# impICNF/ContinuousNF.jl

Measured on AMD Instinct MI355X. Metric: ODE RHS-evals/sec (nvars=32, batch=8192, Tsit5), higher is better.
Workload: dtype f32 (products as six bf16 MFMA terms of exactly split operands, fp32 accumulate); 1 GPU; BASELINE configs[2]: RNODE nvars=32 naugs=0, MLP 32-128-128-32 tanh, batch 8192 per GPU, TrainMode Hutchinson VJP, Tsit5 tspan (0,1), adaptive reltol=sqrt(eps32) abstol=eps32; global_batch=8192, parallelism=columns sharded x1, kernel=mfma

## Files before the change

### continuousnf.jl_amd/csrc/cnf_step3.hip

```cpp
#include "cnf_step3_dev.h"
#include <mutex>

namespace s3 {
constexpr int NB = 32, P0 = 32, PH = 128;
constexpr int SX0 = 40, SXH = 136, SKZ = 264, SW2 = 132;
constexpr int W1T = 0;
constexpr int W3R = W1T + P0 * SXH;
constexpr int X0 = W3R + P0 * SXH;
constexpr int H1 = X0 + NB * SX0;
constexpr int H2 = H1 + NB * SXH;
constexpr int G1 = H2 + NB * SXH;
constexpr int G3 = G1 + NB * SXH;
constexpr int KZ = G3 + NB * SX0;
constexpr int RED = KZ + NB * SKZ;
constexpr int SC = RED + 3 * NB * 8;
constexpr int EPS = SC + NB * 24;
constexpr int BIAS = EPS + NB * SX0;
constexpr int MISC = BIAS + 2 * PH + P0;
constexpr int TOTAL = MISC + 64;
constexpr int STG = X0;
static_assert(STG + PH * SW2 <= RED, "the W2 staging image must not reach the scratch that the prologue uses");
constexpr int IMG_W2 = 0;
constexpr int IMG_W1T = IMG_W2 + PH * SW2;
constexpr int IMG_W3R = IMG_W1T + P0 * SXH;
// ... 1098 lines not shown
            }
            if (live && sown) {
                const f32x4 f1 = read_scalars();
                out[n_in] = f1.x; out[n_in + 1] = f1.y; out[n_in + 2] = f1.z;
                if (a.init_phase >= 0) norms(sc_get(0), sc_get(1), f1, 3);
            }
        }
        if (!single && live && zown) {
            const f32x4 ez = TS_BT1 * kz[0] + TS_BT2 * kz[1] + TS_BT3 * kz[2] + TS_BT4 * kz[3] + TS_BT5 * kz[4] +
                             TS_BT6 * kz[5] + TS_BT7 * kz[6];
#pragma unroll
            for (int c = 0; c < 4; ++c) {
                const float scl = fmaf(fmaxf(fabsf(uz[c]), fabsf(un[c])), reltol, abstol);
                const float x = c < nv ? hstep * ez[c] / scl : 0.f;
                errsum = fmaf(x, x, errsum);
                badcnt += (c < nv && !(fabsf(un[c]) <= 3.0e38f)) ? 1.f : 0.f;
            }
            const size_t gc = (size_t)(tile * 32 + 16 * hf + s) * D;
            if (nv >= 4) { st4_wide(Uout + gc + r0, un); st4_wide(K1out + gc + r0, kz[6]); }
            else { st4(Uout + gc + r0, un, nv); st4(K1out + gc + r0, kz[6], nv); }
        }
        if (!single && live && sown) {
            f32x4 ks[7];
#pragma unroll
            for (int j = 0; j < 6; ++j) ks[j] = sc_get(1 + j);
            const f32x4 us = sc_get(0);
            ks[6] = read_scalars();
            const f32x4 uns = us + hstep * stage_acc4<6>(ks);
            err_acc(errsum, badcnt, ks, us, uns, hstep, abstol, reltol, 3);
            const size_t gc = (size_t)(tile * 32 + 16 * hf + s) * D;
            float* Un = Uout + gc + n_in;
            float* K7 = K1out + gc + n_in;
            Un[0] = uns.x; Un[1] = uns.y; Un[2] = uns.z;
            K7[0] = ks[6].x; K7[1] = ks[6].y; K7[2] = ks[6].z;
        }
        s3_bar();
    }
    errsum = s3_wave_sum(errsum);
    badcnt = s3_wave_sum(badcnt);
    if (lane == 0) { msc[wave] = errsum; msc[16 + wave] = badcnt; }
    s3_bar();
    if (tid == 0) {
        float e = 0.f, b = 0.f;
        for (int w = 0; w < 8; ++w) { e += msc[w]; b += msc[16 + w]; }
        if (!single) {
            a.partials[2 * blockIdx.x] = e;
            a.partials[2 * blockIdx.x + 1] = b;
        } else if (a.init_phase >= 0) {
            __hip_atomic_store(a.partials + 2 * blockIdx.x, e, __ATOMIC_RELAXED, __HIP_MEMORY_SCOPE_AGENT);
            __hip_atomic_store(a.partials + 2 * blockIdx.x + 1, b, __ATOMIC_RELAXED, __HIP_MEMORY_SCOPE_AGENT);
            asm volatile("s_waitcnt vmcnt(0)" ::: "memory");
            const unsigned tk = __hip_atomic_fetch_add(a.ticket, 1u, __ATOMIC_RELAXED, __HIP_MEMORY_SCOPE_AGENT);
            msc[40] = (tk == gridDim.x - 1) ? 1.f : 0.f;
            if (tk == gridDim.x - 1) __hip_atomic_store(a.ticket, 0u, __ATOMIC_RELAXED, __HIP_MEMORY_SCOPE_AGENT);
        }
    }
    if (single && a.init_phase >= 0) {
        s3_bar();
        if (msc[40] != 0.f) {
            float q0 = 0.f, q1 = 0.f;
            for (int i = tid; i < (int)gridDim.x; i += 512) {
                q0 += __hip_atomic_load(a.partials + 2 * i, __ATOMIC_RELAXED, __HIP_MEMORY_SCOPE_AGENT);
                q1 += __hip_atomic_load(a.partials + 2 * i + 1, __ATOMIC_RELAXED, __HIP_MEMORY_SCOPE_AGENT);
            }
            q0 = s3_wave_sum(q0); q1 = s3_wave_sum(q1);
            if (lane == 0) { msc[wave] = q0; msc[16 + wave] = q1; }
            s3_bar();
            if (tid == 0) {
                float p0 = 0.f, p1 = 0.f;
                for (int w = 0; w < 8; ++w) { p0 += msc[w]; p1 += msc[16 + w]; }
                ctrl_phase(a.st_out, single - 1, p0, p1, a.n_total);
            }
        }
    }
}

namespace s3v {
constexpr int SKZ = 264;
constexpr int KZ = 0, RED = KZ + 32 * SKZ, SC = RED + 3 * 32 * 8, BIAS = SC + 32 * 24;
constexpr int MISC = BIAS + 2 * 128 + 32, FP_END = MISC + 64;
constexpr int WS = 256, WP = 32 * WS, WI = 3 * WP;
constexpr int NS = 64, NP = 32 * NS, NI = 3 * NP;
constexpr int H1G = FP_END * 4, H2G = H1G + WI, W3I = H2G + WI, W1TI = W3I + WI, X0S = W1TI + WI, G3S = X0S + NI;
constexpr int TOTAL_BYTES = G3S + NI;
static_assert(H1G % 16 == 0 && TOTAL_BYTES <= 160 * 1024, "LDS plan");
static_assert(WI == s3g::WI, "global image");
}

__global__ void __launch_bounds__(512, 2) k_step3b(MfmaArgs a, const char* __restrict__ imgb, int n_in, int norm_z,
                                                   int norm_j, const S3Tab tab, int single) {
    extern __shared__ __attribute__((aligned(16))) float lds[];
    char* ldsb = reinterpret_cast<char*>(lds);
    const float* img3 = reinterpret_cast<const float*>(imgb);
    S3_ARGS_UP_FRONT(a, imgb);
    const StepState* st = a.st;
    const int tid = threadIdx.x, lane = tid & 63, wave = __builtin_amdgcn_readfirstlane(tid >> 6);
    const int D = n_in + 3;
    const int s = lane & 15, q = lane >> 4;
    const int t = wave & 1, hf = (wave >> 1) & 1;
    const bool zown = wave < 4;
    const bool sown = !zown && t == 0 && q == 0;
    const int smp = 16 * hf + s;
    const int r0 = 16 * t + 4 * q;
    const int nv = n_in - r0;
#ifdef S3_STAMPS
    unsigned long long s3acc[36] = {0};
    unsigned long long s3last = __builtin_amdgcn_s_memtime();
    const unsigned long long s3start = s3last;
#endif
    const StepState* stw = s3_state_words(st);
    const int v_done = stw->done, v_cur = stw->cur;
    const float v_h = stw->h, v_abstol = stw->abstol, v_reltol = stw->reltol;
    const float* ppin = a.apply_ctrl ? a.partials_in : img3;
    const float2 pp = *reinterpret_cast<const float2*>(ppin + 2 * min(tid, (int)gridDim.x - 1));
    const int ntile = (a.B + 32 - 1) / 32;
    const bool wide = (n_in & 3) == 0;
    f32x4 ru[2], rk[2], re, rs[2][2];
    int ce = 0, cu = 0, cs = 0;
    {
        const int b0 = blockIdx.x * 32 + 16 * hf;
        const bool live = s < max(0, min(16, a.B - b0));
        const size_t gcol = (size_t)(b0 + s) * D;
        ce = live ? nv : 0; cu = (zown && live) ? nv : 0; cs = (sown && live) ? 3 : 0;
        re = ld4_issue_w(a.eps + (size_t)(b0 + s) * n_in + r0, ce, img3, wide);
#pragma unroll
        for (int c = 0; c < 2; ++c) {
            ru[c] = ld4_issue_w(a.U[c] + gcol + r0, cu, img3, wide);
            rk[c] = ld4_issue_w(a.K1[c] + gcol + r0, cu, img3, wide);
            rs[c][0] = ld3_issue(a.U[c] + gcol + n_in, cs, img3);
            rs[c][1] = ld3_issue(a.K1[c] + gcol + n_in, cs, img3);
        }
    }
    constexpr int NCI = 2 * s3v::WI / 16, NCB = (2 * 128 + 32) / 4;
    static_assert(NCI % 64 == 0, "whole wave instructions");
    typedef __attribute__((address_space(3))) char* lds_c;
    typedef const __attribute__((address_space(1))) char* glb_c;
    const f32x4 sgb = reinterpret_cast<const f32x4*>(imgb + s3g::BIASB)[min(tid, NCB - 1)];
    S3bOp wF1, wF2[4], wB3, wB2[4];
    {
        const char* fw = imgb + s3g::F32 + (size_t)wave * 10 * 2048 + 16 * lane;
        constexpr int AH = 5;
        f32x4 raw[10][2];
#pragma unroll
        for (int f = 0; f < AH; ++f) { raw[f][0] = *(const f32x4*)(fw + f * 2048); raw[f][1] = *(const f32x4*)(fw + f * 2048 + 1024); }
        __builtin_amdgcn_sched_barrier(0);
#pragma unroll
        for (int f = 0; f < 10; ++f) {
            if (f + AH < 10) {
                raw[f + AH][0] = *(const f32x4*)(fw + (f + AH) * 2048);
                raw[f + AH][1] = *(const f32x4*)(fw + (f + AH) * 2048 + 1024);
            }
            S3bOp o = s3b_split8(raw[f][0], raw[f][1]);
            s3b_pin(o);
            if (f == 0) wF1 = o; else if (f < 5) wF2[f - 1] = o; else if (f == 5) wB3 = o; else wB2[f - 6] = o;
            __builtin_amdgcn_sched_barrier(0);
        }
    }
#pragma unroll
    for (int i = 0; i < (NCI + 511) / 512; ++i) {
        const int c = 512 * i + 64 * wave;
        if (c < NCI)
            __builtin_amdgcn_global_load_lds((glb_c)(imgb + s3g::W3I + 16 * (c + lane)), (lds_c)(ldsb + s3v::W3I + 16 * c), 16, 0, 0);
    }
    float* sc = lds + s3v::SC + smp * 24;
    auto sc_get = [&](int j) { return f32x4{sc[3 * j], sc[3 * j + 1], sc[3 * j + 2], 0.f}; };
    auto sc_set = [&](int j, const f32x4& v) { sc[3 * j] = v.x; sc[3 * j + 1] = v.y; sc[3 * j + 2] = v.z; };
    __builtin_amdgcn_sched_barrier(0);
    S3T(23);
    __builtin_amdgcn_s_waitcnt(0x0F70);
    __builtin_amdgcn_sched_barrier(0);
    S3T(24);
    const int st_done = __builtin_amdgcn_readfirstlane(v_done), st_cur = __builtin_amdgcn_readfirstlane(v_cur);
    const float st_h = __int_as_float(__builtin_amdgcn_readfirstlane(__float_as_int(v_h)));
    const float st_abstol = __int_as_float(__builtin_amdgcn_readfirstlane(__float_as_int(v_abstol)));
    const float st_reltol = __int_as_float(__builtin_amdgcn_readfirstlane(__float_as_int(v_reltol)));
    if (st_done) {
        asm volatile("s_waitcnt vmcnt(0)" ::: "memory");
        if (a.apply_ctrl && blockIdx.x == 0 && tid == 0) { *a.st_out = *st; publish_mirror(a, *st); }
        return;
    }
    if (sown) {
        sc_set(2, ld4_mask(rs[0][0], cs)); sc_set(3, ld4_mask(rs[0][1], cs));
        sc_set(4, ld4_mask(rs[1][0], cs)); sc_set(5, ld4_mask(rs[1][1], cs));
    }
    f32x4 epsr = ld4_mask(re, ce);
    float* msc = lds + s3v::MISC;
    if (a.apply_ctrl) {
        float cp0 = tid < (int)gridDim.x ? pp.x : 0.f, cp1 = tid < (int)gridDim.x ? pp.y : 0.f;
        for (int i = tid + 512; i < (int)gridDim.x; i += 512) { cp0 += a.partials_in[2 * i]; cp1 += a.partials_in[2 * i + 1]; }
        cp0 = s3_wave_sum(cp0); cp1 = s3_wave_sum(cp1);
        if (lane == 0) { msc[wave] = cp0; msc[16 + wave] = cp1; }
    }
    if (tid < NCB) reinterpret_cast<f32x4*>(lds + s3v::BIAS)[tid] = sgb;
    s3_bar();
    S3T(25);
    int cur = st_cur;
    float hstep = st_h, abstol = st_abstol, reltol = st_reltol;
    if (a.apply_ctrl && tid == 0) {
        float p0 = 0.f, p1 = 0.f;
        for (int w = 0; w < 8; ++w) { p0 += msc[w]; p1 += msc[16 + w]; }
        StepState ns = *st;
        ctrl_after_step(&ns, p0, p1, a.n_total);
        if (blockIdx.x == 0) { *a.st_out = ns; publish_mirror(a, ns); }
        msc[32] = __int_as_float(ns.cur); msc[33] = ns.h; msc[34] = ns.abstol; msc[35] = ns.reltol;
        msc[36] = __int_as_float(ns.done);
    }
    S3T(26);
    s3_bar();
    S3T(27);
    if (a.apply_ctrl) {
        cur = __builtin_amdgcn_readfirstlane(__float_as_int(msc[32]));
        hstep = __int_as_float(__builtin_amdgcn_readfirstlane(__float_as_int(msc[33])));
        abstol = __int_as_float(__builtin_amdgcn_readfirstlane(__float_as_int(msc[34])));
        reltol = __int_as_float(__builtin_amdgcn_readfirstlane(__float_as_int(msc[35])));
        if (__float_as_int(msc[36])) return;
    }
    const int nstg = single ? 1 : 6;
    const float c21 = single == 1 ? 0.f : (single == 2 ? 1.f : TS_A21);
    const float* Uin = cur ? a.U[1] : a.U[0];
    const float* K1in = cur ? a.K1[1] : a.K1[0];
    float* Uout = cur ? a.U[0] : a.U[1];
    float* K1out = cur ? a.K1[0] : a.K1[1];

    float errsum = 0.f, badcnt = 0.f;
    auto red8 = [&](int kind) {
        const float* r = lds + s3v::RED + (kind * 32 + smp) * 8;
        const f32x4 a_ = *(const f32x4*)r, b_ = *(const f32x4*)(r + 4);
        return ((a_.x + a_.y) + (a_.z + a_.w)) + ((b_.x + b_.y) + (b_.z + b_.w));
    };
    auto read_scalars = [&]() {
        const float e2 = red8(0), ld = red8(1), n2 = red8(2);
        return f32x4{ld, norm_z ? __builtin_sqrtf(e2) : 0.f, norm_j ? __builtin_sqrtf(n2) : 0.f, 0.f};
    };
    float* redw = lds + s3v::RED + smp * 8 + 4 * t + q;
    const int wb_rd = s * s3v::WS + 16 * (q ^ s);
    const int wb_wr = s * s3v::WS + 16 * ((2 * wave + (q >> 1)) ^ s) + 8 * (q & 1);
    constexpr int HBW = 16 * s3v::WS;
    const char* nrA = ldsb + (zown ? s3v::W3I : s3v::W1TI) + 16 * t * s3v::WS;
    const char* nrB = ldsb + (zown ? s3v::H2G : s3v::H1G) + 16 * hf * s3v::WS;
    const int nsw = (-(s >> 2)) & 3;
    const int nw = smp * s3v::NS + 16 * ((2 * t + (q >> 1)) ^ nsw) + 8 * (q & 1);
    char* x0w = ldsb + s3v::X0S + nw;
    char* g3w = ldsb + s3v::G3S + nw;
    const int nb_rd = s * s3v::NS + 16 * (q ^ nsw);
    constexpr int HBN = 16 * s3v::NS;
    float* rkw = lds + s3v::KZ + smp * s3v::SKZ + r0;
    float* kzw = rkw + 64;
    const float* bias = lds + s3v::BIAS;
    const f32x4 zero4 = {0.f, 0.f, 0.f, 0.f};

    S3T(20);
    auto tile_in = [&](const f32x4& uz, f32x4 k1z) {
        if (single == 1) { k1z = zero4; if (sown) sc_set(1, k1z); }
        if (zown) {
            s3b_store4(x0w, s3v::NP, uz + (hstep * c21) * k1z);
            *(f32x4*)rkw = uz;
            *(f32x4*)(rkw + 32) = k1z;
#pragma unroll
            for (int j = 0; j < 6; ++j) *(f32x4*)(kzw + 32 * j) = zero4;
        }
    };
    if (sown) { sc_set(0, sc_get(cur ? 4 : 2)); sc_set(1, sc_get(cur ? 5 : 3)); }
    tile_in(ld4_mask(cur ? ru[1] : ru[0], cu), ld4_mask(cur ? rk[1] : rk[0], cu));
    for (int tile = blockIdx.x; tile < ntile; tile += gridDim.x) {
        const int b0 = tile * 32 + 16 * hf;
        const bool live = s < max(0, min(16, a.B - b0));
        const size_t gcol = (size_t)(b0 + s) * D;
        if (tile != (int)blockIdx.x) {
            ce = live ? nv : 0; cu = (zown && live) ? nv : 0; cs = (sown && live) ? 3 : 0;
            const f32x4 e_ = ld4_issue_w(a.eps + (size_t)(b0 + s) * n_in + r0, ce, img3, wide);
            const f32x4 u_ = ld4_issue_w(Uin + gcol + r0, cu, img3, wide), k_ = ld4_issue_w(K1in + gcol + r0, cu, img3, wide);
            const f32x4 s0 = ld3_issue(Uin + gcol + n_in, cs, img3), s1 = ld3_issue(K1in + gcol + n_in, cs, img3);
            epsr = ld4_mask(e_, ce);
            if (sown) { sc_set(0, ld4_mask(s0, cs)); sc_set(1, ld4_mask(s1, cs)); }
            tile_in(ld4_mask(u_, cu), ld4_mask(k_, cu));
        }
        s3_bar();
        S3T(21);

        constexpr bool S3B_RECORDS = false;
        constexpr bool S3B_COND = false;
        float* const dmpw = nullptr; const size_t dmp_stride = 0;
        (void)dmpw; (void)dmp_stride;
#include "cnf_step3b_eval.inc"
        if (single) {
            float* out = (single == 1 ? a.du : a.Ks0) + (size_t)(tile * 32 + 16 * hf + s) * D;
            auto norms = [&](const f32x4& u4, const f32x4& f0, const f32x4& f1, int nvalid) {
#pragma unroll
                for (int c = 0; c < 4; ++c) {
                    if (c < nvalid) {
                        const float sk = fmaf(fabsf(u4[c]), reltol, abstol);
                        if (single == 1) {
                            const float x = u4[c] / sk, y = f1[c] / sk;
                            errsum = fmaf(x, x, errsum); badcnt = fmaf(y, y, badcnt);
                        } else {
                            const float x = (f1[c] - f0[c]) / sk;
                            errsum = fmaf(x, x, errsum);
                        }
                    }
                }
            };
            if (live && zown) {
                const f32x4 f1 = *(const f32x4*)kzw;
                st4(out + r0, f1, nv);
                if (a.init_phase >= 0) norms(*(const f32x4*)rkw, *(const f32x4*)(rkw + 32), f1, nv);
            }
            if (live && sown) {
                const f32x4 f1 = read_scalars();
                out[n_in] = f1.x; out[n_in + 1] = f1.y; out[n_in + 2] = f1.z;
                if (a.init_phase >= 0) norms(sc_get(0), sc_get(1), f1, 3);
            }
        }
        if (!single && live && zown) {
            const f32x4 k7z = *(const f32x4*)(kzw + 32 * 5), uz_ = *(const f32x4*)rkw;
            const f32x4 un = s3b_load4(x0w, s3v::NP);
            f32x4 ez = TS_BT1 * *(const f32x4*)(rkw + 32) + TS_BT7 * k7z;
            ez += TS_BT2 * *(const f32x4*)(kzw) + TS_BT3 * *(const f32x4*)(kzw + 32) + TS_BT4 * *(const f32x4*)(kzw + 64) +
                  TS_BT5 * *(const f32x4*)(kzw + 96) + TS_BT6 * *(const f32x4*)(kzw + 128);
#pragma unroll
            for (int c = 0; c < 4; ++c) {
                const float scl = fmaf(fmaxf(fabsf(uz_[c]), fabsf(un[c])), reltol, abstol);
                const float x = c < nv ? hstep * ez[c] / scl : 0.f;
                errsum = fmaf(x, x, errsum);
                badcnt += (c < nv && !(fabsf(un[c]) <= 3.0e38f)) ? 1.f : 0.f;
            }
            const size_t gc = (size_t)(tile * 32 + 16 * hf + s) * D;
            float* Un = Uout + gc + r0;
            float* K7 = K1out + gc + r0;
            if (nv >= 4) { st4_wide(Un, un); st4_wide(K7, k7z); }
            else { st4(Un, un, nv); st4(K7, k7z, nv); }
        }
        if (!single && live && sown) {
            f32x4 ks[7];
#pragma unroll
            for (int j = 0; j < 6; ++j) ks[j] = sc_get(1 + j);
            const f32x4 us = sc_get(0);
            ks[6] = read_scalars();
            const f32x4 uns = us + hstep * stage_acc4<6>(ks);
            err_acc(errsum, badcnt, ks, us, uns, hstep, abstol, reltol, 3);
            const size_t gc = (size_t)(tile * 32 + 16 * hf + s) * D;
            float* Un = Uout + gc + n_in;
            float* K7 = K1out + gc + n_in;
            Un[0] = uns.x; Un[1] = uns.y; Un[2] = uns.z;
            K7[0] = ks[6].x; K7[1] = ks[6].y; K7[2] = ks[6].z;
// ... 150 lines not shown
    const char* nrA = ldsb + (zown ? s3v::W3I : s3v::W1TI) + 16 * t * s3v::WS;
    const char* nrB = ldsb + (zown ? s3v::H2G : s3v::H1G) + 16 * hf * s3v::WS;
    const int nsw = (-(s >> 2)) & 3;
    const int nw = smp * s3v::NS + 16 * ((2 * t + (q >> 1)) ^ nsw) + 8 * (q & 1);
    char* x0w = ldsb + s3v::X0S + nw;
    char* g3w = ldsb + s3v::G3S + nw;
    const int nb_rd = s * s3v::NS + 16 * (q ^ nsw);
    constexpr int HBN = 16 * s3v::NS;
    float* rkw = lds + s3v::KZ + smp * s3v::SKZ + r0;
    float* kzw = rkw + 64;
    const float* bias = lds + s3v::BIAS;
    const f32x4 zero4 = {0.f, 0.f, 0.f, 0.f};

    if (zown) { *(f32x4*)rkw = ld4_mask(ru, cu); *(f32x4*)(rkw + 32) = zero4; }
    if (sown) { sc_set(0, ld4_mask(rs, cs)); sc_set(1, zero4); }
    s3_bar();
    float hstep = ns->h, abstol = ns->abstol, reltol = ns->reltol;
    hstep = __int_as_float(__builtin_amdgcn_readfirstlane(__float_as_int(hstep)));
    abstol = __int_as_float(__builtin_amdgcn_readfirstlane(__float_as_int(abstol)));
    reltol = __int_as_float(__builtin_amdgcn_readfirstlane(__float_as_int(reltol)));
    int nsync = 0;
    const unsigned mbase = __builtin_amdgcn_readfirstlane(__hip_atomic_load(sv.base_dev, __ATOMIC_RELAXED, __HIP_MEMORY_SCOPE_AGENT));
    auto meet = [&](float e_lane, float b_lane) -> bool {
        float e = s3_wave_sum(e_lane), b = s3_wave_sum(b_lane);
        if (lane == 0) { msc[wave] = e; msc[16 + wave] = b; }
        s3_bar();
        unsigned long long* pb = reinterpret_cast<unsigned long long*>(sv.part) + (nsync & 1) * 1024;
        const unsigned tag = mbase + (unsigned)nsync + 1u;
        if (tid == 0) {
            float e8 = 0.f, b8 = 0.f;
            for (int w = 0; w < 8; ++w) { e8 += msc[w]; b8 += msc[16 + w]; }
            __hip_atomic_store(pb + 2 * blockIdx.x, ((unsigned long long)tag << 32) | __float_as_uint(e8), __ATOMIC_RELAXED,
                               __HIP_MEMORY_SCOPE_AGENT);
            __hip_atomic_store(pb + 2 * blockIdx.x + 1, ((unsigned long long)tag << 32) | __float_as_uint(b8), __ATOMIC_RELAXED,
                               __HIP_MEMORY_SCOPE_AGENT);
        }
        float cp0 = 0.f, cp1 = 0.f;
        int ok = 1;
        if (tid < (int)gridDim.x) {
            ok = 0;
            const unsigned long long wait0 = __builtin_amdgcn_s_memrealtime();
            for (int spin = 0; spin < sv.spin_limit; ++spin) {
                u32x4 wq;
                asm volatile("global_load_dwordx4 %0, %1, off sc0 sc1\n\ts_waitcnt vmcnt(0)" : "=v"(wq) : "v"(pb + 2 * tid) : "memory");
                const unsigned long long w0 = ((unsigned long long)wq.y << 32) | wq.x, w1 = ((unsigned long long)wq.w << 32) | wq.z;
                if ((unsigned)(w0 >> 32) == tag && (unsigned)(w1 >> 32) == tag) {
                    cp0 = __uint_as_float((unsigned)w0); cp1 = __uint_as_float((unsigned)w1); ok = 1;
                    break;
                }
                if ((spin & 255) == 255 && __hip_atomic_load(sv.abort_flag, __ATOMIC_RELAXED, __HIP_MEMORY_SCOPE_AGENT)) break;
                if ((spin & 15) == 15 && __builtin_amdgcn_s_memrealtime() - wait0 > sv.wait_ticks) break;
                __builtin_amdgcn_s_sleep(4);
            }
            if (!ok) __hip_atomic_store(sv.abort_flag, 1, __ATOMIC_RELAXED, __HIP_MEMORY_SCOPE_AGENT);
        }
        cp0 = s3_wave_sum(cp0); cp1 = s3_wave_sum(cp1);
        const float bad = s3_wave_sum(ok ? 0.f : 1.f);
        s3_bar();
        if (lane == 0) { msc[wave] = cp0; msc[16 + wave] = cp1; msc[24 + wave] = bad; }
        s3_bar();
        float nbad = 0.f;
        for (int w = 0; w < 8; ++w) nbad += msc[24 + w];
        if (tid == 0) {
            float p0 = 0.f, p1 = 0.f;
            for (int w = 0; w < 8; ++w) { p0 += msc[w]; p1 += msc[16 + w]; }
            msc[32] = p0; msc[33] = p1;
        }
        ++nsync;
        return nbad == 0.f;
    };
    auto share = [&]() {
        s3_bar();
        hstep = __int_as_float(__builtin_amdgcn_readfirstlane(__float_as_int(msc[36])));
        abstol = __int_as_float(__builtin_amdgcn_readfirstlane(__float_as_int(msc[37])));
        reltol = __int_as_float(__builtin_amdgcn_readfirstlane(__float_as_int(msc[38])));
        const int fl = __builtin_amdgcn_readfirstlane(__float_as_int(msc[39]));
        s3_bar();
        return fl;
    };
    auto post_ctrl = [&](int accepted) {
        msc[36] = ns->h; msc[37] = ns->abstol; msc[38] = ns->reltol;
        msc[39] = __int_as_float((ns->done ? 1 : 0) | (accepted ? 2 : 0));
    };
    int nstg = 1;
    float* dmpw = nullptr;
    const size_t dmp_stride = a.dump_stride;
    auto evals = [&]() {
        constexpr bool S3B_RECORDS = RECORD;
        constexpr bool S3B_COND = COND;
#include "cnf_step3b_eval.inc"
    };
    auto add_norm = [&](float& acc, float u, float x) {
        const float sk = fmaf(fabsf(u), reltol, abstol);
        const float y = x / sk;
        acc = fmaf(y, y, acc);
    };
    int cur = 0;
    auto load_tile = [&](int tile, bool with_k1, bool from_xs) {
        set_tile(tile);
        const float* Uc = cur ? a.U[1] : a.U[0];
        const float* Kc = cur ? a.K1[1] : a.K1[0];
        const f32x4 e_ = ld4_issue_w(a.eps + (size_t)(b0 + s) * n_in + r0, ce, img3, wide);
        f32x4 u_, s_;
        if (from_xs) {
            const float* xc = sv.xs + (size_t)(b0 + s) * sv.nvars;
#pragma unroll
            for (int j = 0; j < 4; ++j) u_[j] = (cu > j && r0 + j < sv.nvars) ? xc[r0 + j] : 0.f;
            s_ = zero4;
        } else {
            u_ = ld4_issue_w(Uc + gcol + r0, cu, img3, wide);
            s_ = ld3_issue(Uc + gcol + n_in, cs, img3);
        }
        f32x4 k_ = zero4, ks_ = zero4;
        if (with_k1) { k_ = ld4_issue_w(Kc + gcol + r0, cu, img3, wide); ks_ = ld3_issue(Kc + gcol + n_in, cs, img3); }
        epsr = ld4_mask(e_, ce);
        if (zown) { *(f32x4*)rkw = ld4_mask(u_, cu); *(f32x4*)(rkw + 32) = ld4_mask(k_, cu); }
        if (sown) { sc_set(0, ld4_mask(s_, cs)); sc_set(1, ld4_mask(ks_, cs)); }
    };
    auto store_rows = [&](float* dst, const f32x4& z4, const f32x4& s4) {
        if (live && zown) { if (nv >= 4) st4_wide(dst + gcol + r0, z4); else st4(dst + gcol + r0, z4, nv); }
        if (live && sown) { float* o = dst + gcol + n_in; o[0] = s4.x; o[1] = s4.y; o[2] = s4.z; }
    };
    bool alive = true;
    {
        float e = 0.f, b = 0.f;
        for (int tile = blockIdx.x; tile < ntile; tile += gridDim.x) {
            if (multi) { load_tile(tile, false, sv.xs != nullptr); }
            if (zown) {
                s3b_store4(x0w, s3v::NP, *(const f32x4*)rkw);
#pragma unroll
                for (int j = 0; j < 6; ++j) *(f32x4*)(kzw + 32 * j) = zero4;
            }
            s3_bar();
            nstg = 1; evals();
            f32x4 f0z = zero4, f0s = zero4;
            if (zown) f0z = *(const f32x4*)kzw;
            if (live && zown) {
                const f32x4 u4 = *(const f32x4*)rkw;
#pragma unroll
                for (int c = 0; c < 4; ++c) if (c < nv) { add_norm(e, u4[c], u4[c]); add_norm(b, u4[c], f0z[c]); }
            }
            if (zown) *(f32x4*)(rkw + 32) = f0z;
            if (sown) f0s = read_scalars();
            if (live && sown) {
                const f32x4 u4 = sc_get(0);
#pragma unroll
                for (int c = 0; c < 3; ++c) { add_norm(e, u4[c], u4[c]); add_norm(b, u4[c], f0s[c]); }
            }
            if (sown) sc_set(1, f0s);
            if (multi) {
                if (sv.xs) store_rows(a.U[0], zown ? *(const f32x4*)rkw : zero4, sown ? sc_get(0) : zero4);
                store_rows(a.K1[0], f0z, f0s);
                s3_bar();
            }
        }
        if (sv.hairer) alive = meet(e, b);
        if (sv.hairer && alive) {
            if (tid == 0) { ctrl_phase(ns, 0, msc[32], msc[33], a.n_total); post_ctrl(0); }
            share();
            e = 0.f; b = 0.f;
            for (int tile = blockIdx.x; tile < ntile; tile += gridDim.x) {
                if (multi) { load_tile(tile, true, false); }
                if (zown) {
                    s3b_store4(x0w, s3v::NP, *(const f32x4*)rkw + hstep * *(const f32x4*)(rkw + 32));
#pragma unroll
                    for (int j = 0; j < 6; ++j) *(f32x4*)(kzw + 32 * j) = zero4;
                }
                s3_bar();
                nstg = 1; evals();
                if (live && zown) {
                    const f32x4 u4 = *(const f32x4*)rkw, f0 = *(const f32x4*)(rkw + 32), f1 = *(const f32x4*)kzw;
#pragma unroll
                    for (int c = 0; c < 4; ++c) if (c < nv) add_norm(e, u4[c], f1[c] - f0[c]);
                }
                if (live && sown) {
                    const f32x4 u4 = sc_get(0), f0 = sc_get(1), f1 = read_scalars();
#pragma unroll
                    for (int c = 0; c < 3; ++c) add_norm(e, u4[c], f1[c] - f0[c]);
                }
                if (multi) s3_bar();
            }
            alive = meet(e, b);
            if (alive) {
                if (tid == 0) { ctrl_phase(ns, 1, msc[32], msc[33], a.n_total); post_ctrl(0); }
                share();
            }
        }
    }
    int done = 0;
    int nacc = 0;
    if (wave < 4) __builtin_amdgcn_s_setprio(1);
    for (int it = 0; alive && !done && it < sv.maxiters; ++it) {
      float errsum = 0.f, badcnt = 0.f;
      for (int tile = blockIdx.x; tile < ntile; tile += gridDim.x) {
        if (multi) { load_tile(tile, true, false); }
        if (zown) {
            const f32x4 u2 = *(const f32x4*)rkw + (hstep * TS_A21) * *(const f32x4*)(rkw + 32);
            s3b_store4(x0w, s3v::NP, u2);
#pragma unroll
            for (int j = 0; j < 6; ++j) *(f32x4*)(kzw + 32 * j) = zero4;
            if (RECORD) {
                dmpw = (live && nacc < a.dump_cap) ? a.dump + (size_t)nacc * a.dump_step_stride + gcol + r0 : nullptr;
                if (dmpw && nv > 0) {
                    const f32x4 un_ = *(const f32x4*)rkw;
                    if (nv >= 4) { st4_wide(dmpw - dmp_stride, un_); st4_wide(dmpw, u2); }
                    else { st4(dmpw - dmp_stride, un_, nv); st4(dmpw, u2, nv); }
                }
            }
        }
        if (RECORD && blockIdx.x == 0 && tid == 0 && nacc < a.dump_cap) a.hs_out[nacc] = hstep;
        s3_bar();
        nstg = 6; evals();
        if (live && zown) {
            const f32x4 k7z = *(const f32x4*)(kzw + 32 * 5), uz_ = *(const f32x4*)rkw;
            const f32x4 un = s3b_load4(x0w, s3v::NP);
            f32x4 ez = TS_BT1 * *(const f32x4*)(rkw + 32) + TS_BT7 * k7z;
            ez += TS_BT2 * *(const f32x4*)(kzw) + TS_BT3 * *(const f32x4*)(kzw + 32) + TS_BT4 * *(const f32x4*)(kzw + 64) +
                  TS_BT5 * *(const f32x4*)(kzw + 96) + TS_BT6 * *(const f32x4*)(kzw + 128);
#pragma unroll
            for (int c = 0; c < 4; ++c) {
                const float scl = fmaf(fmaxf(fabsf(uz_[c]), fabsf(un[c])), reltol, abstol);
                const float x = c < nv ? hstep * ez[c] / scl : 0.f;
                errsum = fmaf(x, x, errsum);
                badcnt += (c < nv && !(fabsf(un[c]) <= 3.0e38f)) ? 1.f : 0.f;
            }
        }
        f32x4 uns = zero4, k7s = zero4;
        if (sown) {
            f32x4 ks[7];
#pragma unroll
            for (int j = 0; j < 6; ++j) ks[j] = sc_get(1 + j);
            const f32x4 us = sc_get(0);
            ks[6] = read_scalars();
            k7s = ks[6];
            uns = us + hstep * stage_acc4<6>(ks);
            if (live) err_acc(errsum, badcnt, ks, us, uns, hstep, abstol, reltol, 3);
            sc_set(7, uns);
        }
        if (multi) {
            float* Un = cur ? a.U[0] : a.U[1];
            float* Kn = cur ? a.K1[0] : a.K1[1];
            store_rows(Un, zown ? s3b_load4(x0w, s3v::NP) : zero4, uns);
            store_rows(Kn, zown ? *(const f32x4*)(kzw + 32 * 5) : zero4, k7s);
            s3_bar();
        }
      }
        alive = meet(errsum, badcnt);
        if (!alive) break;
        if (tid == 0) {
            const int acc0 = ns->naccept;
            const float t_att = ns->t, h_att = ns->h;
            ctrl_after_step(ns, msc[32], msc[33], a.n_total);
            post_ctrl(ns->naccept != acc0);
            if (sv.trace && blockIdx.x == 0 && it < sv.trace_cap)
                *(f32x4u*)(sv.trace + 4 * it) = f32x4{t_att, h_att, ns->eest, ns->naccept != acc0 ? 1.f : 0.f};
        }
        const int fl = share();
        done = fl & 1;
        if (fl & 2 && multi) { ++nacc; cur ^= 1; }
        else if (fl & 2) {
            ++nacc;
            if (zown) {
                *(f32x4*)rkw = s3b_load4(x0w, s3v::NP);
                *(f32x4*)(rkw + 32) = *(const f32x4*)(kzw + 32 * 5);
            }
            if (sown) { const f32x4 k7s = read_scalars(); sc_set(0, sc_get(7)); sc_set(1, k7s); }
        }
    }
    if (!multi && (alive || !sv.u_out)) store_rows(sv.u_out ? sv.u_out : a.U[0], zown ? *(const f32x4*)rkw : zero4, sown ? sc_get(0) : zero4);
    float v4[4] = {0.f, 0.f, 0.f, 0.f};
    if (sv.logpx && alive) {
      for (int tile = blockIdx.x; tile < ntile; tile += gridDim.x) {
        if (multi) {
            set_tile(tile);
            const float* Uc = cur ? a.U[1] : a.U[0];
            const f32x4 u_ = ld4_issue_w(Uc + gcol + r0, cu, img3, wide), s_ = ld3_issue(Uc + gcol + n_in, cs, img3);
            s3_bar();
            if (zown) *(f32x4*)rkw = ld4_mask(u_, cu);
            if (sown) sc_set(0, ld4_mask(s_, cs));
        }
        if (zown) {
            const f32x4 u4 = *(const f32x4*)rkw;
            float ss = 0.f, sa = 0.f;
#pragma unroll
            for (int c = 0; c < 4; ++c)
                if (c < nv) { ss = fmaf(u4[c], u4[c], ss); if (r0 + c >= sv.nvars) sa = fmaf(u4[c], u4[c], sa); }
            redw[0] = ss; redw[32 * 8] = sa;
        }
        s3_bar();
        if (live && sown) {
            const float ss = red8(0), sa = red8(1);
            const f32x4 us = sc_get(0);
            const float log2pi = 1.8378770664093453f;
            const float lp = -0.5f * fmaf((float)n_in, log2pi, ss) - us.x;
            const float aa = (sv.norm_z_aug && sv.naugs > 0) ? sqrtf(sa) : 0.f;
            const size_t b = (size_t)(b0 + s), Bz = (size_t)a.B;
            sv.logpx[b] = lp; sv.regs[b] = us.y; sv.regs[Bz + b] = us.z; sv.regs[2 * Bz + b] = aa;
            v4[0] += lp; v4[1] += us.y; v4[2] += us.z; v4[3] += aa;
        }
      }
        if (sv.sums5) {
            unsigned long long* qb = reinterpret_cast<unsigned long long*>(sv.part) + 2048;
            const unsigned tag = mbase + (unsigned)nsync + 1u;
#pragma unroll
            for (int j = 0; j < 4; ++j) v4[j] = s3_wave_sum(v4[j]);
            s3_bar();
            if (lane == 0 && (wave == 4 || wave == 6)) for (int j = 0; j < 4; ++j) msc[(wave == 4 ? 0 : 8) + j] = v4[j];
            s3_bar();
            if (tid < 4)
                __hip_atomic_store(qb + 4 * blockIdx.x + tid, ((unsigned long long)tag << 32) | __float_as_uint(msc[tid] + msc[8 + tid]),
                                   __ATOMIC_RELAXED, __HIP_MEMORY_SCOPE_AGENT);
            if (blockIdx.x == 0) {
                float c4[4] = {0.f, 0.f, 0.f, 0.f};
                float late = 0.f;
                if (tid < (int)gridDim.x) {
#pragma unroll
                    for (int j = 0; j < 4; ++j) {
                        int got = 0;
                        const unsigned long long wait0 = __builtin_amdgcn_s_memrealtime();
                        for (int spin = 0; spin < sv.spin_limit; ++spin) {
                            const unsigned long long w = __hip_atomic_load(qb + 4 * tid + j, __ATOMIC_RELAXED, __HIP_MEMORY_SCOPE_AGENT);
                            if ((unsigned)(w >> 32) == tag) { c4[j] = __uint_as_float((unsigned)w); got = 1; break; }
                            if ((spin & 15) == 15 && __builtin_amdgcn_s_memrealtime() - wait0 > sv.wait_ticks) break;
                            __builtin_amdgcn_s_sleep(1);
                        }
                        if (!got) late = 1.f;
                    }
                    if (late != 0.f) __hip_atomic_store(sv.abort_flag, 1, __ATOMIC_RELAXED, __HIP_MEMORY_SCOPE_AGENT);
                }
#pragma unroll
                for (int j = 0; j < 4; ++j) c4[j] = s3_wave_sum(c4[j]);
                late = s3_wave_sum(late);
                s3_bar();
                if (lane == 0) { for (int j = 0; j < 4; ++j) msc[4 * wave + j] = c4[j]; msc[32 + wave] = late; }
                s3_bar();
                if (tid < 4) {
                    float r = 0.f;
                    for (int w = 0; w < 8; ++w) r += msc[4 * w + tid];
                    sv.sums5[tid] = r;
                }
                if (tid == 0) {
                    sv.sums5[4] = (float)a.B;
                    float nl = 0.f;
                    for (int w = 0; w < 8; ++w) nl += msc[32 + w];
                    if (nl != 0.f) { ns->done = 0; ns->n_partials = -1; }
                }
            }
        }
    }
    if (blockIdx.x == 0 && tid == 0) {
        if (!alive || __hip_atomic_load(sv.abort_flag, __ATOMIC_RELAXED, __HIP_MEMORY_SCOPE_AGENT)) { ns->done = 0; ns->n_partials = -1; }
// ... 634 lines not shown
```

### continuousnf.jl_amd/csrc/cnf_step3_dev.h

```cpp
#pragma once
#include "cnf_step3.h"
#include "cnf_split.h"

struct S3Tab { float a[7][8]; };
static const S3Tab kS3Tab = {{
    {0, 0, 0, 0, 0, 0, 0, 0},
    {TS_A21, 0, 0, 0, 0, 0, 0, 0},
    {TS_A31, TS_A32, 0, 0, 0, 0, 0, 0},
    {TS_A41, TS_A42, TS_A43, 0, 0, 0, 0, 0},
    {TS_A51, TS_A52, TS_A53, TS_A54, 0, 0, 0, 0},
    {TS_A61, TS_A62, TS_A63, TS_A64, TS_A65, 0, 0, 0},
    {TS_A71, TS_A72, TS_A73, TS_A74, TS_A75, TS_A76, 0, 0}}};

#define S3_SB() __builtin_amdgcn_sched_barrier(0)
__device__ __forceinline__ void s3_bar() {
    __builtin_amdgcn_sched_barrier(0);
#ifdef S3_ABL_NOBAR
    asm volatile("s_waitcnt lgkmcnt(0)" ::: "memory");
#else
    asm volatile("s_waitcnt lgkmcnt(0)\n\ts_barrier" ::: "memory");
#endif
    __builtin_amdgcn_sched_barrier(0);
}

// ... 16 lines not shown
    v += __int_as_float(__builtin_amdgcn_mov_dpp(__float_as_int(v), 0xB1, 0xF, 0xF, true));
    v += __int_as_float(__builtin_amdgcn_mov_dpp(__float_as_int(v), 0x4E, 0xF, 0xF, true));
    v += __int_as_float(__builtin_amdgcn_mov_dpp(__float_as_int(v), 0x141, 0xF, 0xF, true));
    v += __int_as_float(__builtin_amdgcn_mov_dpp(__float_as_int(v), 0x140, 0xF, 0xF, true));
    const int i = __float_as_int(v);
    return (__int_as_float(__builtin_amdgcn_readlane(i, 0)) + __int_as_float(__builtin_amdgcn_readlane(i, 16))) +
           (__int_as_float(__builtin_amdgcn_readlane(i, 32)) + __int_as_float(__builtin_amdgcn_readlane(i, 48)));
}

namespace s3g {
constexpr int BIASB = 0;
constexpr int F32 = (2 * 128 + 32) * 4;
constexpr int NFR = 8 * 10 + 2 * 4;
constexpr int W3I = F32 + NFR * 2048;
constexpr int WI = 3 * 32 * 256;
constexpr int IMG_BYTES = W3I + 2 * WI;
static_assert(F32 % 16 == 0 && W3I % 16 == 0, "16-byte loads");
}

typedef unsigned u32x2_ __attribute__((ext_vector_type(2)));
__device__ __forceinline__ void s3b_store4(char* img, int piece_bytes, const f32x4& v) {
#ifdef S3_ABL_NOSTORE
    { asm volatile("" :: "v"(v), "v"((unsigned)(size_t)img)); return; }
#endif
    u32x2_ h, m, l;
    { unsigned h_, m_, l_; s3b_split2(v[0], v[1], h_, m_, l_); h.x = h_; m.x = m_; l.x = l_; }
    { unsigned h_, m_, l_; s3b_split2(v[2], v[3], h_, m_, l_); h.y = h_; m.y = m_; l.y = l_; }
    *(u32x2_*)img = h; *(u32x2_*)(img + piece_bytes) = m; *(u32x2_*)(img + 2 * piece_bytes) = l;
}
struct S3bOp { bf16x8 h, m, l; };
__device__ __forceinline__ S3bOp s3b_load(const char* img, int piece_bytes) {
    S3bOp o;
#ifdef S3_ABL_NOLOAD
    { typedef unsigned u4_ __attribute__((ext_vector_type(4))); u4_ z = {0x3c003c00u, 0x3c003c00u, 0x3c003c00u, 0x3c003c00u}; asm volatile("" : "+v"(z) : "v"((unsigned)(size_t)img));
      o.h = o.m = o.l = __builtin_bit_cast(bf16x8, z); return o; }
#endif
    o.h = *(const bf16x8*)img; o.m = *(const bf16x8*)(img + piece_bytes); o.l = *(const bf16x8*)(img + 2 * piece_bytes);
    return o;
}
typedef unsigned u32x4 __attribute__((ext_vector_type(4)));
__device__ __forceinline__ S3bOp s3b_split8(const f32x4& lo4, const f32x4& hi4) {
    u32x4 h, m, l;
    { unsigned h_, m_, l_; s3b_split2(lo4[0], lo4[1], h_, m_, l_); h.x = h_; m.x = m_; l.x = l_; }
    { unsigned h_, m_, l_; s3b_split2(lo4[2], lo4[3], h_, m_, l_); h.y = h_; m.y = m_; l.y = l_; }
    { unsigned h_, m_, l_; s3b_split2(hi4[0], hi4[1], h_, m_, l_); h.z = h_; m.z = m_; l.z = l_; }
    { unsigned h_, m_, l_; s3b_split2(hi4[2], hi4[3], h_, m_, l_); h.w = h_; m.w = m_; l.w = l_; }
    S3bOp o;
    o.h = __builtin_bit_cast(bf16x8, h); o.m = __builtin_bit_cast(bf16x8, m); o.l = __builtin_bit_cast(bf16x8, l);
    return o;
}
__device__ __forceinline__ void s3b_pin(S3bOp& o) {
    u32x4 a = __builtin_bit_cast(u32x4, o.h), b = __builtin_bit_cast(u32x4, o.m), c = __builtin_bit_cast(u32x4, o.l);
    asm volatile("" : "+v"(a), "+v"(b), "+v"(c));
    o.h = __builtin_bit_cast(bf16x8, a); o.m = __builtin_bit_cast(bf16x8, b); o.l = __builtin_bit_cast(bf16x8, c);
}
template <int T>
__device__ __forceinline__ f32x4 s3b_term(const S3bOp& a, const S3bOp& b, const f32x4& acc) {
#ifdef S3_ABL_NOMFMA
    { u32x4 x = __builtin_bit_cast(u32x4, a.h), y = __builtin_bit_cast(u32x4, b.h); asm volatile("" :: "v"(x), "v"(y)); return acc; }
#endif
    if (T == 0) return __builtin_amdgcn_mfma_f32_16x16x32_bf16(a.l, b.h, acc, 0, 0, 0);
    if (T == 1) return __builtin_amdgcn_mfma_f32_16x16x32_bf16(a.h, b.l, acc, 0, 0, 0);
    if (T == 2) return __builtin_amdgcn_mfma_f32_16x16x32_bf16(a.m, b.m, acc, 0, 0, 0);
    if (T == 3) return __builtin_amdgcn_mfma_f32_16x16x32_bf16(a.m, b.h, acc, 0, 0, 0);
    if (T == 4) return __builtin_amdgcn_mfma_f32_16x16x32_bf16(a.h, b.m, acc, 0, 0, 0);
    return __builtin_amdgcn_mfma_f32_16x16x32_bf16(a.h, b.h, acc, 0, 0, 0);
}
template <int NC>
__device__ __forceinline__ void s3b_mm(f32x4 (&acc)[NC], const S3bOp& a, const S3bOp (&b)[NC]) {
#pragma unroll
    for (int n = 0; n < NC; ++n) acc[n] = s3b_term<0>(a, b[n], acc[n]);
#pragma unroll
    for (int n = 0; n < NC; ++n) acc[n] = s3b_term<1>(a, b[n], acc[n]);
#pragma unroll
    for (int n = 0; n < NC; ++n) acc[n] = s3b_term<2>(a, b[n], acc[n]);
#pragma unroll
    for (int n = 0; n < NC; ++n) acc[n] = s3b_term<3>(a, b[n], acc[n]);
#pragma unroll
    for (int n = 0; n < NC; ++n) acc[n] = s3b_term<4>(a, b[n], acc[n]);
#pragma unroll
    for (int n = 0; n < NC; ++n) acc[n] = s3b_term<5>(a, b[n], acc[n]);
}

__device__ __forceinline__ f32x4 s3b_load4(const char* img, int piece_bytes) {
    const bf16x4 h = *(const bf16x4*)img, m = *(const bf16x4*)(img + piece_bytes), l = *(const bf16x4*)(img + 2 * piece_bytes);
    f32x4 v;
#pragma unroll
    for (int j = 0; j < 4; ++j) v[j] = (float)h[j] + ((float)m[j] + (float)l[j]);
    return v;
}
```

### continuousnf.jl_amd/csrc/cnf_step3b_eval.inc

```
        for (int stg = 1; stg <= nstg; ++stg) {
            f32x4 d2a, d2b;
            {
                f32x4 bv1 = *(const f32x4*)(bias + 16 * wave + 4 * q), bv1b = bv1;
                if (S3B_COND) {
                    const int tb = b0 - 16 * hf;
                    bv1 = *(const f32x4*)(a.cond + (size_t)min(tb + s, a.B - 1) * a.cbs + 16 * wave + 4 * q);
                    bv1b = *(const f32x4*)(a.cond + (size_t)min(tb + 16 + s, a.B - 1) * a.cbs + 16 * wave + 4 * q);
                }
                S3bOp b[2];
                b[0] = s3b_load(ldsb + s3v::X0S + nb_rd, s3v::NP);
                b[1] = s3b_load(ldsb + s3v::X0S + nb_rd + HBN, s3v::NP);
                S3_SB();
                f32x4 acc[2] = {zero4, zero4};
                s3b_mm<2>(acc, wF1, b);
                s3b_store4(ldsb + s3v::H1G + wb_wr, s3v::WP, s3_tanh4(acc[0] + bv1));
                s3b_store4(ldsb + s3v::H1G + wb_wr + HBW, s3v::WP, s3_tanh4(acc[1] + bv1b));
            }
            S3T(0);
            s3_bar();
            S3T(1);
            {
                const f32x4 bv2 = *(const f32x4*)(bias + 128 + 16 * wave + 4 * q);
                if (stg > 1 && sown) sc_set(stg, read_scalars());
                f32x4 acc[2] = {zero4, zero4};
#pragma unroll
                for (int kb = 0; kb < 4; ++kb) {
                    S3bOp b[2];
                    b[0] = s3b_load(ldsb + s3v::H1G + (wb_rd ^ (64 * kb)), s3v::WP);
                    b[1] = s3b_load(ldsb + s3v::H1G + HBW + (wb_rd ^ (64 * kb)), s3v::WP);
                    S3_SB();
                    s3b_mm<2>(acc, wF2[kb], b);
                    S3_SB();
                }
                const f32x4 h2a = s3_tanh4(acc[0] + bv2), h2b = s3_tanh4(acc[1] + bv2);
                d2a = s3_dtanh4(h2a); d2b = s3_dtanh4(h2b);
                s3b_store4(ldsb + s3v::H2G + wb_wr, s3v::WP, h2a);
                s3b_store4(ldsb + s3v::H2G + wb_wr + HBW, s3v::WP, h2b);
            }
            S3T(2);
            s3_bar();
            S3T(3);
            if (zown) {
                const f32x4 bv3 = *(const f32x4*)(bias + 256 + r0);
                f32x4 z0 = zero4, z1 = zero4;
#pragma unroll
                for (int kb = 0; kb < 4; ++kb) {
                    const S3bOp av = s3b_load(nrA + (wb_rd ^ (64 * kb)), s3v::WP), bvv = s3b_load(nrB + (wb_rd ^ (64 * kb)), s3v::WP);
                    S3_SB();
                    z0 = s3b_term<0>(av, bvv, z0); z1 = s3b_term<3>(av, bvv, z1);
                    z0 = s3b_term<1>(av, bvv, z0); z1 = s3b_term<4>(av, bvv, z1);
                    z0 = s3b_term<2>(av, bvv, z0); z1 = s3b_term<5>(av, bvv, z1);
                    S3_SB();
                }
                const float* A = tab.a[stg < 6 ? stg + 1 : 6];
                f32x4 pre = *(const f32x4*)rkw + (hstep * A[0]) * *(const f32x4*)(rkw + 32);
#pragma unroll
                for (int j = 1; j < 5; ++j) pre += (hstep * A[j]) * *(const f32x4*)(kzw + 32 * (j - 1));
                const f32x4 zd = s3_tanh4(z0 + z1 + bv3);
                s3b_store4(g3w, s3v::NP, epsr * s3_dtanh4(zd));
                const f32x4 xnext = pre + (hstep * A[stg]) * zd;
                if (stg < 6) s3b_store4(x0w, s3v::NP, xnext);
                if (S3B_RECORDS && dmpw && stg < 5 && nv > 0) { if (nv >= 4) st4_wide(dmpw + (size_t)stg * dmp_stride, xnext); else st4(dmpw + (size_t)stg * dmp_stride, xnext, nv); }
                *(f32x4*)(kzw + 32 * (stg - 1)) = zd;
                redw[0] = s3_dot4(zd, zd);
            }
            S3T(4);
            s3_bar();
            S3T(5);
            {
                S3bOp b[2];
                b[0] = s3b_load(ldsb + s3v::G3S + nb_rd, s3v::NP);
                b[1] = s3b_load(ldsb + s3v::G3S + nb_rd + HBN, s3v::NP);
                S3_SB();
                f32x4 acc[2] = {zero4, zero4};
                s3b_mm<2>(acc, wB3, b);
                s3b_store4(ldsb + s3v::H2G + wb_wr, s3v::WP, acc[0] * d2a);
                s3b_store4(ldsb + s3v::H2G + wb_wr + HBW, s3v::WP, acc[1] * d2b);
            }
            S3T(6);
            s3_bar();
            S3T(7);
            {
                const f32x4 h1a = s3b_load4(ldsb + s3v::H1G + wb_wr, s3v::WP), h1b = s3b_load4(ldsb + s3v::H1G + wb_wr + HBW, s3v::WP);
                f32x4 acc[2] = {zero4, zero4};
#pragma unroll
                for (int kb = 0; kb < 4; ++kb) {
                    S3bOp b[2];
                    b[0] = s3b_load(ldsb + s3v::H2G + (wb_rd ^ (64 * kb)), s3v::WP);
                    b[1] = s3b_load(ldsb + s3v::H2G + HBW + (wb_rd ^ (64 * kb)), s3v::WP);
                    S3_SB();
                    s3b_mm<2>(acc, wB2[kb], b);
                    S3_SB();
                }
                s3b_store4(ldsb + s3v::H1G + wb_wr, s3v::WP, acc[0] * s3_dtanh4(h1a));
                s3b_store4(ldsb + s3v::H1G + wb_wr + HBW, s3v::WP, acc[1] * s3_dtanh4(h1b));
            }
            S3T(8);
            s3_bar();
            S3T(9);
            if (!zown) {
                f32x4 j0 = zero4, j1 = zero4;
#pragma unroll
                for (int kb = 0; kb < 4; ++kb) {
                    const S3bOp av = s3b_load(nrA + (wb_rd ^ (64 * kb)), s3v::WP), bvv = s3b_load(nrB + (wb_rd ^ (64 * kb)), s3v::WP);
                    S3_SB();
                    j0 = s3b_term<0>(av, bvv, j0); j1 = s3b_term<3>(av, bvv, j1);
                    j0 = s3b_term<1>(av, bvv, j0); j1 = s3b_term<4>(av, bvv, j1);
                    j0 = s3b_term<2>(av, bvv, j0); j1 = s3b_term<5>(av, bvv, j1);
                    S3_SB();
                }
                const f32x4 ej = j0 + j1;
                redw[32 * 8] = -s3_dot4(ej, epsr);
                redw[2 * 32 * 8] = s3_dot4(ej, ej);
            }
            S3T(10);
            s3_bar();
            S3T(11);
        }
```

Baseline: 174,300 RHS-evals/s.

## Precompute next-stage RK combination during idle phase and software-pipeline narrow MFMA loads

The Runge-Kutta stage prefix sum (u + h*sum a_j k_j) moves off the critical path after the forward third layer. The z-owning waves now precompute it into an LDS slot while the other waves run the Jacobian narrow product, and h-scaled tableau rows are staged in LDS. The narrow 32x32 MFMA loop becomes a shared helper that double-buffers operand loads so LDS reads overlap the bf16 MFMA terms. This costs extra LDS, a few more registers and a changed stage-index convention (nstg, cz), which could affect correctness or occupancy.

```diff
diff --git a/continuousnf.jl_amd/csrc/cnf_step3.hip b/continuousnf.jl_amd/csrc/cnf_step3.hip
--- a/continuousnf.jl_amd/csrc/cnf_step3.hip
+++ b/continuousnf.jl_amd/csrc/cnf_step3.hip
@@ -1204,8 +1204,9 @@
 constexpr int WS = 256, WP = 32 * WS, WI = 3 * WP;
 constexpr int NS = 64, NP = 32 * NS, NI = 3 * NP;
 constexpr int H1G = FP_END * 4, H2G = H1G + WI, W3I = H2G + WI, W1TI = W3I + WI, X0S = W1TI + WI, G3S = X0S + NI;
-constexpr int TOTAL_BYTES = G3S + NI;
-static_assert(H1G % 16 == 0 && TOTAL_BYTES <= 160 * 1024, "LDS plan");
+constexpr int PRES = G3S + NI, HAT = PRES + 256 * 16;
+constexpr int TOTAL_BYTES = HAT + 8 * 8 * 4;
+static_assert(H1G % 16 == 0 && PRES % 16 == 0 && TOTAL_BYTES <= 160 * 1024, "LDS plan");
 static_assert(WI == s3g::WI, "global image");
 }
 
@@ -1372,6 +1373,30 @@
     const f32x4 zero4 = {0.f, 0.f, 0.f, 0.f};
 
     S3T(20);
+    float* prew = reinterpret_cast<float*>(ldsb + s3v::PRES) + 4 * (tid & 255);
+    float* hat = reinterpret_cast<float*>(ldsb + s3v::HAT);
+    float cz = 0.f;
+    auto s3b_fill_hat = [&]() {
+        if (wave >= 4 && lane == 0) {
+            f32x4 lo, hi;
+#pragma unroll
+            for (int j = 0; j < 4; ++j) { lo[j] = hstep * tab.a[wave - 1][j]; hi[j] = hstep * tab.a[wave - 1][4 + j]; }
+            *(f32x4*)(hat + 8 * (wave - 1)) = lo; *(f32x4*)(hat + 8 * (wave - 1) + 4) = hi;
+        }
+    };
+    auto s3b_pre_first = [&]() {
+        const float c[5] = {hstep * tab.a[2][0], hstep * tab.a[2][1], hstep * tab.a[2][2], hstep * tab.a[2][3], hstep * tab.a[2][4]};
+        *(f32x4*)prew = s3b_stage_pre(rkw, c);
+        cz = __int_as_float(__builtin_amdgcn_readfirstlane(__float_as_int(c[1])));
+    };
+    auto s3b_pre_next = [&](int e) {
+        const float* row = hat + 8 * (e + 1);
+        const f32x4 lo = *(const f32x4*)row;
+        const float c[5] = {lo.x, lo.y, lo.z, lo.w, row[4]};
+        const float ce_ = row[e];
+        *(f32x4*)prew = s3b_stage_pre(rkw, c);
+        cz = __int_as_float(__builtin_amdgcn_readfirstlane(__float_as_int(ce_)));
+    };
     auto tile_in = [&](const f32x4& uz, f32x4 k1z) {
         if (single == 1) { k1z = zero4; if (sown) sc_set(1, k1z); }
         if (zown) {
@@ -1380,8 +1405,10 @@
             *(f32x4*)(rkw + 32) = k1z;
 #pragma unroll
             for (int j = 0; j < 6; ++j) *(f32x4*)(kzw + 32 * j) = zero4;
-        }
-    };
+            s3b_pre_first();
+        }
+    };
+    s3b_fill_hat();
     if (sown) { sc_set(0, sc_get(cur ? 4 : 2)); sc_set(1, sc_get(cur ? 5 : 3)); }
     tile_in(ld4_mask(cur ? ru[1] : ru[0], cu), ld4_mask(cur ? rk[1] : rk[0], cu));
     for (int tile = blockIdx.x; tile < ntile; tile += gridDim.x) {
@@ -1698,6 +1725,30 @@
         msc[36] = ns->h; msc[37] = ns->abstol; msc[38] = ns->reltol;
         msc[39] = __int_as_float((ns->done ? 1 : 0) | (accepted ? 2 : 0));
     };
+    float* prew = reinterpret_cast<float*>(ldsb + s3v::PRES) + 4 * (tid & 255);
+    float* hat = reinterpret_cast<float*>(ldsb + s3v::HAT);
+    float cz = 0.f;
+    auto s3b_fill_hat = [&]() {
+        if (wave >= 4 && lane == 0) {
+            f32x4 lo, hi;
+#pragma unroll
+            for (int j = 0; j < 4; ++j) { lo[j] = hstep * tab.a[wave - 1][j]; hi[j] = hstep * tab.a[wave - 1][4 + j]; }
+            *(f32x4*)(hat + 8 * (wave - 1)) = lo; *(f32x4*)(hat + 8 * (wave - 1) + 4) = hi;
+        }
+    };
+    auto s3b_pre_first = [&]() {
+        const float c[5] = {hstep * tab.a[2][0], hstep * tab.a[2][1], hstep * tab.a[2][2], hstep * tab.a[2][3], hstep * tab.a[2][4]};
+        *(f32x4*)prew = s3b_stage_pre(rkw, c);
+        cz = __int_as_float(__builtin_amdgcn_readfirstlane(__float_as_int(c[1])));
+    };
+    auto s3b_pre_next = [&](int e) {
+        const float* row = hat + 8 * (e + 1);
+        const f32x4 lo = *(const f32x4*)row;
+        const float c[5] = {lo.x, lo.y, lo.z, lo.w, row[4]};
+        const float ce_ = row[e];
+        *(f32x4*)prew = s3b_stage_pre(rkw, c);
+        cz = __int_as_float(__builtin_amdgcn_readfirstlane(__float_as_int(ce_)));
+    };
     int nstg = 1;
     float* dmpw = nullptr;
     const size_t dmp_stride = a.dump_stride;
@@ -1815,6 +1866,7 @@
             s3b_store4(x0w, s3v::NP, u2);
 #pragma unroll
             for (int j = 0; j < 6; ++j) *(f32x4*)(kzw + 32 * j) = zero4;
+            s3b_pre_first();
             if (RECORD) {
                 dmpw = (live && nacc < a.dump_cap) ? a.dump + (size_t)nacc * a.dump_step_stride + gcol + r0 : nullptr;
                 if (dmpw && nv > 0) {
@@ -1825,6 +1877,7 @@
             }
         }
         if (RECORD && blockIdx.x == 0 && tid == 0 && nacc < a.dump_cap) a.hs_out[nacc] = hstep;
+        s3b_fill_hat();
         s3_bar();
         nstg = 6; evals();
         if (live && zown) {
@@ -1883,6 +1936,14 @@
             if (sown) { const f32x4 k7s = read_scalars(); sc_set(0, sc_get(7)); sc_set(1, k7s); }
         }
     }
+#ifdef S3_STAMPS
+    if (blockIdx.x == 7 && lane == 0 && (wave == 0 || wave == 5)) {
+        unsigned long long tot = 0;
+        for (int i = 0; i < 12; ++i) tot += s3acc[i];
+        printf("k_solve3b wave %d total %llu | F1 %llu+%llu F2 %llu+%llu F3 %llu+%llu B3 %llu+%llu B2 %llu+%llu B1 %llu+%llu\n", wave, tot,
+               s3acc[0], s3acc[1], s3acc[2], s3acc[3], s3acc[4], s3acc[5], s3acc[6], s3acc[7], s3acc[8], s3acc[9], s3acc[10], s3acc[11]);
+    }
+#endif
     if (!multi && (alive || !sv.u_out)) store_rows(sv.u_out ? sv.u_out : a.U[0], zown ? *(const f32x4*)rkw : zero4, sown ? sc_get(0) : zero4);
     float v4[4] = {0.f, 0.f, 0.f, 0.f};
     if (sv.logpx && alive) {
diff --git a/continuousnf.jl_amd/csrc/cnf_step3_dev.h b/continuousnf.jl_amd/csrc/cnf_step3_dev.h
--- a/continuousnf.jl_amd/csrc/cnf_step3_dev.h
+++ b/continuousnf.jl_amd/csrc/cnf_step3_dev.h
@@ -122,6 +122,35 @@
     for (int n = 0; n < NC; ++n) acc[n] = s3b_term<5>(a, b[n], acc[n]);
 }
 
+__device__ __forceinline__ void s3b_narrow(const char* A, const char* B, int rd, int piece_bytes, f32x4& c0, f32x4& c1) {
+    S3bOp av[2], bv[2];
+    av[0] = s3b_load(A + rd, piece_bytes); bv[0] = s3b_load(B + rd, piece_bytes);
+    S3_SB();
+#pragma unroll
+    for (int kb = 0; kb < 4; ++kb) {
+        const int cb = kb & 1, nb = cb ^ 1;
+        if (kb < 3) { av[nb] = s3b_load(A + (rd ^ (64 * (kb + 1))), piece_bytes); bv[nb] = s3b_load(B + (rd ^ (64 * (kb + 1))), piece_bytes); }
+        S3_SB();
+        c0 = s3b_term<0>(av[cb], bv[cb], c0); c1 = s3b_term<3>(av[cb], bv[cb], c1);
+        S3_SB();
+        c0 = s3b_term<1>(av[cb], bv[cb], c0); c1 = s3b_term<4>(av[cb], bv[cb], c1);
+        S3_SB();
+        c0 = s3b_term<2>(av[cb], bv[cb], c0); c1 = s3b_term<5>(av[cb], bv[cb], c1);
+        S3_SB();
+    }
+}
+
+__device__ __forceinline__ f32x4 s3b_stage_pre(const float* rk, const float (&c)[5]) {
+    const f32x4 u = *(const f32x4*)rk, k1 = *(const f32x4*)(rk + 32);
+    f32x4 pre = {fmaf(c[0], k1.x, u.x), fmaf(c[0], k1.y, u.y), fmaf(c[0], k1.z, u.z), fmaf(c[0], k1.w, u.w)};
+#pragma unroll
+    for (int j = 1; j < 5; ++j) {
+        const f32x4 k = *(const f32x4*)(rk + 64 + 32 * (j - 1));
+        pre = f32x4{fmaf(c[j], k.x, pre.x), fmaf(c[j], k.y, pre.y), fmaf(c[j], k.z, pre.z), fmaf(c[j], k.w, pre.w)};
+    }
+    return pre;
+}
+
 __device__ __forceinline__ f32x4 s3b_load4(const char* img, int piece_bytes) {
     const bf16x4 h = *(const bf16x4*)img, m = *(const bf16x4*)(img + piece_bytes), l = *(const bf16x4*)(img + 2 * piece_bytes);
     f32x4 v;
diff --git a/continuousnf.jl_amd/csrc/cnf_step3b_eval.inc b/continuousnf.jl_amd/csrc/cnf_step3b_eval.inc
--- a/continuousnf.jl_amd/csrc/cnf_step3b_eval.inc
+++ b/continuousnf.jl_amd/csrc/cnf_step3b_eval.inc
@@ -42,25 +42,16 @@
             S3T(3);
             if (zown) {
                 const f32x4 bv3 = *(const f32x4*)(bias + 256 + r0);
+                const f32x4 pre = *(const f32x4*)prew;
                 f32x4 z0 = zero4, z1 = zero4;
-#pragma unroll
-                for (int kb = 0; kb < 4; ++kb) {
-                    const S3bOp av = s3b_load(nrA + (wb_rd ^ (64 * kb)), s3v::WP), bvv = s3b_load(nrB + (wb_rd ^ (64 * kb)), s3v::WP);
-                    S3_SB();
-                    z0 = s3b_term<0>(av, bvv, z0); z1 = s3b_term<3>(av, bvv, z1);
-                    z0 = s3b_term<1>(av, bvv, z0); z1 = s3b_term<4>(av, bvv, z1);
-                    z0 = s3b_term<2>(av, bvv, z0); z1 = s3b_term<5>(av, bvv, z1);
-                    S3_SB();
-                }
-                const float* A = tab.a[stg < 6 ? stg + 1 : 6];
-                f32x4 pre = *(const f32x4*)rkw + (hstep * A[0]) * *(const f32x4*)(rkw + 32);
-#pragma unroll
-                for (int j = 1; j < 5; ++j) pre += (hstep * A[j]) * *(const f32x4*)(kzw + 32 * (j - 1));
+                s3b_narrow(nrA, nrB, wb_rd, s3v::WP, z0, z1);
                 const f32x4 zd = s3_tanh4(z0 + z1 + bv3);
                 s3b_store4(g3w, s3v::NP, epsr * s3_dtanh4(zd));
-                const f32x4 xnext = pre + (hstep * A[stg]) * zd;
-                if (stg < 6) s3b_store4(x0w, s3v::NP, xnext);
-                if (S3B_RECORDS && dmpw && stg < 5 && nv > 0) { if (nv >= 4) st4_wide(dmpw + (size_t)stg * dmp_stride, xnext); else st4(dmpw + (size_t)stg * dmp_stride, xnext, nv); }
+                if (stg < nstg) {
+                    const f32x4 xnext = {fmaf(cz, zd.x, pre.x), fmaf(cz, zd.y, pre.y), fmaf(cz, zd.z, pre.z), fmaf(cz, zd.w, pre.w)};
+                    s3b_store4(x0w, s3v::NP, xnext);
+                    if (S3B_RECORDS && dmpw && stg < 5 && nv > 0) { if (nv >= 4) st4_wide(dmpw + (size_t)stg * dmp_stride, xnext); else st4(dmpw + (size_t)stg * dmp_stride, xnext, nv); }
+                }
                 *(f32x4*)(kzw + 32 * (stg - 1)) = zd;
                 redw[0] = s3_dot4(zd, zd);
             }
@@ -100,18 +91,12 @@
             S3T(9);
             if (!zown) {
                 f32x4 j0 = zero4, j1 = zero4;
-#pragma unroll
-                for (int kb = 0; kb < 4; ++kb) {
-                    const S3bOp av = s3b_load(nrA + (wb_rd ^ (64 * kb)), s3v::WP), bvv = s3b_load(nrB + (wb_rd ^ (64 * kb)), s3v::WP);
-                    S3_SB();
-                    j0 = s3b_term<0>(av, bvv, j0); j1 = s3b_term<3>(av, bvv, j1);
-                    j0 = s3b_term<1>(av, bvv, j0); j1 = s3b_term<4>(av, bvv, j1);
-                    j0 = s3b_term<2>(av, bvv, j0); j1 = s3b_term<5>(av, bvv, j1);
-                    S3_SB();
-                }
+                s3b_narrow(nrA, nrB, wb_rd, s3v::WP, j0, j1);
                 const f32x4 ej = j0 + j1;
                 redw[32 * 8] = -s3_dot4(ej, epsr);
                 redw[2 * 32 * 8] = s3_dot4(ej, ej);
+            } else if (stg + 1 < nstg) {
+                s3b_pre_next(stg + 1);
             }
             S3T(10);
             s3_bar();
```

After: 174,400 RHS-evals/s (median of 5 runs). About the same (+0.0%).
